# harrywaugh/UOB_Raytracer

Measured on AMD Instinct MI355X. Metric: Mrays/sec (nominal = W*H*AA*(1+S)/t), Cornell Box 4096^2, 8xAA, 64 shadow rays, higher is better.
Workload: dtype f32; 1 GPU; headline: Cornell Box 4096x4096, 4x2 AA, 64 shadow rays, 2 spheres, <=10 bounces, 26 triangles; parallelism=1 GPU

## Files before the change

include/uob_rt.h:

```cpp
#ifndef UOB_RT_H
#define UOB_RT_H

#include <stddef.h>
#include <stdint.h>

#ifdef __cplusplus
extern "C" {
#endif

#define RT_ABI_VERSION 2
#define RT_MAX_SPHERES 4
#define RT_MAX_DEVICES 8

enum {
  RT_OK = 0,
  RT_E_INVALID = -1,
  RT_E_DEVICE = -2,
  RT_E_NOMEM = -3,
  RT_E_IO = -4,
  RT_E_UNSUPPORTED = -5
};

typedef struct rt_sphere {
  float center[3];
// ... 197 lines not shown
int rt_debug_block_costs(rt_ctx* ctx, uint32_t* out, int32_t cap);

int rt_debug_world_masks(rt_ctx* ctx, uint64_t* out, int64_t cap, int32_t* grid, int32_t* words);

int rt_debug_tile_data(rt_ctx* ctx, int32_t* orig, float* tiles, int32_t cap_tiles);

int rt_debug_scene_data(rt_ctx* ctx, float* vertices4, float* normals4, float* colors4, float* vertices4_m,
                        float* normals4_m, float* colors4_m, int32_t* n_shadow, float vbox_lo[3], float vbox_hi[3],
                        int32_t cap_triangles);

int rt_register_output(rt_ctx* ctx, void* host, size_t bytes);
int rt_unregister_output(rt_ctx* ctx);

int rt_debug_wave_timeline(rt_ctx* ctx, uint64_t out[8]);

int rt_debug_wave_seeds(rt_ctx* ctx, void* records, int64_t cap, int32_t dims[3], uint64_t counters[4]);

int rt_debug_wave_seeds_wide(rt_ctx* ctx, void* records, int64_t cap, int32_t dims[3], uint64_t counters[10]);

enum { RT_COPY_2D = 0,
       RT_COPY_PEER = 1,
       RT_COPY_LINEAR = 2    };
typedef struct rt_band_copy {
  int32_t op, reserved;
  uint64_t dst_offset, dst_pitch, src_offset, src_pitch, width_bytes, rows;
} rt_band_copy;
int rt_debug_band_copy_plan(int32_t num_devices, int32_t k, int32_t device_band_rows, int32_t width, int32_t height,
                            int32_t elem_bytes, int32_t dev_to_dev, int32_t peer_ok, int32_t same_device,
                            rt_band_copy* out, int32_t cap);

// ... 35 lines not shown
```

uob_raytracer_amd/csrc/rt_api.hip:

```cpp
#include <cmath>
#include <cstdarg>
#include <cstdio>
#include <cstdlib>
#include <cstring>
#include <memory>
#include <new>
#include <string>
#include <vector>

#include "rt_host.h"

namespace uobrt {

static thread_local std::string g_last_error;

void set_error(const char* fmt, ...) {
  char buf[1024];
  va_list ap;
  va_start(ap, fmt);
  vsnprintf(buf, sizeof buf, fmt, ap);
  va_end(ap);
  g_last_error = buf;
}

// ... 306 lines not shown
  const float zero3[3] = {0.f, 0.f, 0.f}, ident[12] = {1, 0, 0, 0, 0, 1, 0, 0, 0, 0, 1, 0};
  fill_params(c, ident, zero3, light, 1.0f, P);
  if (tiled) use_tiled_scene(c, P);
}

enum class Family { wave, mesh, generic };

static bool frame_cull(const rt_ctx* c) { return !(c->cfg.flags & RT_FLAG_NO_CULL); }

static Family frame_family(const rt_ctx* c, const FrameParams& P) {
  if (c->cfg.flags & RT_FLAG_GENERIC_KERNEL) return Family::generic;
  if (wave_kernel_supports(P) && (frame_cull(c) || P.aa_x * P.aa_y <= 64)) return Family::wave;
  return frame_cull(c) && mesh_kernel_supports(P) ? Family::mesh : Family::generic;
}

static void attach_heavy_lists(rt_ctx* c, FrameParams* P) {
  if (!c->d_heavy_flags || P->job_tasks < 4) return;
  const int prev = c->heavy_phase, cur = prev ^ 1;
  unsigned int* const st[2] = {c->d_jobctr, c->d_jobctr + (2 * kJobHeads + 1) * kJobHeadStride};
  P->heavy_prev = c->d_heavy[prev]; P->heavy_prev_state = st[prev];
  P->heavy_new = c->d_heavy[cur]; P->heavy_new_state = st[cur];
  P->heavy_flags = c->d_heavy_flags + (size_t)prev * c->heavy_jobs_max; P->heavy_flags_new = c->d_heavy_flags + (size_t)cur * c->heavy_jobs_max;
  P->heavy_gen = ++c->heavy_gen;
  P->heavy_factor4 = c->tune.heavy_factor4;
  P->heavy_cap = P->njobs / 3 < c->heavy_cap ? P->njobs / 3 : c->heavy_cap;
  P->heavy_dilate = c->tune.heavy_dilate ? 1 : 0;
  c->heavy_phase = cur;
}

static int attach_timeline(rt_ctx* c, hipStream_t stream, FrameParams* P) {
  c->timeline_valid = false;
  if (!c->tune.timeline) return RT_OK;
  const size_t waves = (size_t)P->wave_blocks * 4;
  if (!c->d_timeline) {
    if (c->d_timeline.alloc(waves * 3) != hipSuccess) { set_error("hipMalloc failed (timeline)"); return RT_E_NOMEM; }
    c->timeline_waves = waves;
  }
  if (c->timeline_waves >= waves) {
    HIP_TRY(hipMemsetAsync(c->d_timeline, 0, c->timeline_waves * 3 * sizeof(uint64_t), stream));
    P->counters = reinterpret_cast<unsigned long long*>(c->d_timeline.p);
    c->timeline_valid = true;
  }
// ... 26 lines not shown
    }
  if (!(fabsf(focal) <= 1.0e9f)) { set_error("focal length must be finite and <= 1e9"); return RT_E_INVALID; }
  for (int k = 0; k < 12; ++k)
    if (!(fabsf(rot[k]) <= 4.0f)) { set_error("rotation matrix entries must be finite and <= 4"); return RT_E_INVALID; }
  if (c->owned_rows == 0) return RT_OK;
  FrameParams P;
  fill_params(c, rot, cam, light, focal, &P);
  P.out_argb = d_argb; P.out_rgb = d_rgb; P.counters = nullptr;
  P.out_global = out_global ? 1 : 0;
  HIP_TRY(hipSetDevice(c->device));
  if (c->timed && stream != c->last_stream) HIP_TRY(hipStreamWaitEvent(stream, c->ev1, 0));
  HIP_TRY(wait_aov(c, stream));
  HIP_TRY(wait_scene(c, stream));
  HIP_TRY(hipEventRecord(c->ev0, stream));
  c->seed_tile_rows = 0;
  const Family family = frame_family(c, P);
  if (family == Family::wave) {
    attach_heavy_lists(c, &P);
    int rc = attach_timeline(c, stream, &P);
    if (rc == RT_OK) rc = attach_seeds(c, rot, &P);
    if (rc != RT_OK) return rc;
    launch_wave(P, frame_cull(c), false, false, stream);
  } else if (family == Family::mesh) {
    use_tiled_scene(c, &P);
    if (c->d_mesh_cost) {
      P.mesh_order = c->mesh_order_valid ? c->d_mesh_order : nullptr;
      P.mesh_cost = c->d_mesh_cost; P.mesh_order_out = c->d_mesh_order;
      P.mesh_queue_len = c->d_mesh_order + 4 * (size_t)((c->cfg.width + 15) / 16) * (size_t)((c->owned_rows + 15) / 16);
      c->mesh_order_valid = true;
    }
    launch_stage_records(P, stream);
    launch_mesh(P, false, false, stream, c->aux_stream, c->ev_fork, c->ev_join);
  } else {
    launch_generic(P, false, stream);
// ... 273 lines not shown
  HIP_TRY(hipMemcpy(rec.data(), c->d_timeline, rec.size() * sizeof(uint64_t), hipMemcpyDeviceToHost));
  for (int q = 0; q < 8; ++q) out[q] = 0;
  out[1] = ~0ull;
  for (size_t w = 0; w < c->timeline_waves; ++w) {
    const uint64_t t0 = rec[3 * w], t1 = rec[3 * w + 1], jobs = rec[3 * w + 2] & 0xffffffffull;
    if (t1 == 0) continue;
    out[7] = rec[3 * w + 2] >> 32;
    out[0] += 1; out[3] += t0; out[4] += t1; out[5] += jobs;
    if (t0 < out[1]) out[1] = t0;
    if (t1 > out[2]) out[2] = t1;
    if (jobs > out[6]) out[6] = jobs;
  }
  return RT_OK;
}

static int seed_table_view(rt_ctx* c, void* records, int64_t cap, int32_t dims[3], uint64_t* counters, int ncounters,
                           void (*view)(SeedRec& r, uint64_t rows, uint64_t* counters)) {
  if (!c || !dims || !counters || cap < 0 || (cap > 0 && !records)) { set_error("NULL argument"); return RT_E_INVALID; }
  c = lead_ctx(c);
  dims[0] = c->seed_tile_rows; dims[1] = c->seed_nseg; dims[2] = c->seed_rows;
  for (int q = 0; q < ncounters; ++q) counters[q] = 0;
  if (c->seed_tile_rows == 0) { dims[1] = 0; return RT_OK; }
  DeviceGuard guard;
  HIP_TRY(hipSetDevice(c->device));
  if (c->timed) HIP_TRY(hipEventSynchronize(c->ev1));
  std::vector<SeedRec> rec((size_t)c->seed_tile_rows * (size_t)c->seed_nseg);
  HIP_TRY(hipMemcpy(rec.data(), c->d_seed, rec.size() * sizeof(SeedRec), hipMemcpyDeviceToHost));
  const rt_config& g = c->cfg;
  for (int tr = 0; tr < c->seed_tile_rows; ++tr) {
    uint64_t rows = 0;
// ... 155 lines not shown
```

uob_raytracer_amd/csrc/rt_device.h:

```cpp
#pragma once
#include <hip/hip_runtime.h>
#include <stdint.h>

#include "../../include/uob_rt.h"

namespace uobrt {

constexpr int kJobHeads = 31;
constexpr int kJobHeadStride = 32;
constexpr int kHeavyStateWords = 8;
constexpr float kMaxCoordinate = 65536.0f;
constexpr int kRecordsPerTriangle = 8;

struct DevSphere {
  float cx, cy, cz, r2;
  float col[4];
};

struct alignas(16) SeedRec {
  float D0[3], ed;
  unsigned long long K, Kh, Kp;
  int32_t h;
  uint32_t flags;
  uint32_t pad[4];
};
// ... 101 lines not shown
```

uob_raytracer_amd/csrc/rt_host.h:

```cpp
#pragma once
#include <hip/hip_runtime.h>

#include <atomic>
#include <string>
#include <utility>
#include <vector>

#include "rt_device.h"

#define HIP_TRY(expr)                                                                   \
  do {                                                                                  \
    hipError_t e_ = (expr);                                                             \
    if (e_ != hipSuccess) {                                                             \
      uobrt::set_error("%s failed: %s (%s:%d)", #expr, hipGetErrorString(e_), __FILE__, __LINE__); \
      return RT_E_DEVICE;                                                               \
    }                                                                                   \
  } while (0)

namespace uobrt {

void set_error(const char* fmt, ...);

struct KeepError {
  std::string text;
// ... 1 lines not shown
  ~KeepError();
};

constexpr int kMaxTriangles = 4000000;
constexpr int kWorldGrid = 32;

void launch_generic(const FrameParams& P, bool count, hipStream_t stream);
bool generic_needs_records(int n);
void launch_stage_records(const FrameParams& P, hipStream_t stream);
void launch_trace_rays(const FrameParams& P, int what, const float* d_rays, const float* d_r2, long nray, int* d_tri,
                       float* d_out10, hipStream_t stream);
void launch_wave(const FrameParams& P, bool cull, bool count, bool prof, hipStream_t stream);
bool wave_kernel_supports(const FrameParams& P);
bool wave_takes_seed(const FrameParams& P, bool cull);
bool wave_can_count(const FrameParams& P, bool cull);
int wave_blocks_per_cu(bool leave_room);
void launch_mesh(const FrameParams& P, bool count, bool prof, hipStream_t stream, hipStream_t aux, hipEvent_t ev_fork, hipEvent_t ev_join);
void launch_bin_primary(const FrameParams& P, hipStream_t stream);
bool mesh_kernel_supports(const FrameParams& P);
int mesh_tiles(int n);
int mesh_occ_words(int grid);
int mesh_screen_cells(int pixels);
int mesh_blocks_per_cu();
int launch_scene_check(const float4* v, const float4* col, int n, unsigned int* out, hipStream_t stream);
void launch_scene_refit(const float4* v, const float4* nrm, const float4* col, const int* orig, int n, float4* vm, float4* nm,
                        float4* cm, float4* tile_box, hipStream_t stream);
constexpr unsigned int kPoseStatic = 0xffffu;
void launch_pose(const float4* rest_v, const float4* rest_n, const unsigned short* object_of, const float* d_xforms12, int n,
                 float4* out_v, float4* out_n, hipStream_t stream);
void launch_skin(const float4* rest_v, const float4* rest_n, const ushort4* index, const float4* weights, const float* d_bones12,
// ... 149 lines not shown
  int cap = 0;
  uobrt::SceneStore own;
  uobrt::DevBuffer tile_scratch;
  int owned_rows = 0;
  uobrt::DevMem<float4> d_verts, d_normals, d_colors;
  uobrt::DevMem<uint32_t> d_argb;
  uobrt::DevMem<float4> d_rgb;
  uobrt::DevMem<unsigned long long> d_counters;
  uobrt::DevMem<unsigned int> d_jobctr;
  uobrt::DevMem<uobrt::SeedRec> d_seed;
  size_t seed_cap = 0;
  int seed_tile_rows = 0, seed_nseg = 0, seed_rows = 0;
  int cus = 256;
  unsigned int *d_heavy[2] = {nullptr, nullptr}, *d_heavy_flags = nullptr;
  int heavy_cap = 0, heavy_phase = 0;
  size_t heavy_jobs_max = 0;
  char* reg_host = nullptr; char* reg_dev = nullptr; size_t reg_bytes = 0;
  bool reg_owner = false;
  bool timeline_valid = false;
  uobrt::DevMem<uint64_t> d_timeline;
  size_t timeline_waves = 0;
  uint32_t heavy_gen = 0;
  float4* d_records = nullptr;
  float4 *d_verts_m = nullptr, *d_normals_m = nullptr, *d_colors_m = nullptr, *d_tile_box = nullptr;
  int* d_orig = nullptr;
  uobrt::DevMem<uobrt::DevSphere> d_spheres;
  unsigned int *d_mesh_cost = nullptr, *d_mesh_order = nullptr;
  bool mesh_order_valid = false;
  unsigned long long *d_screen_masks = nullptr, *d_world_masks = nullptr;
  unsigned int* d_world_occ = nullptr;
// ... 71 lines not shown
```

uob_raytracer_amd/csrc/rt_kernel_wave.hip:

```cpp
#define RT_SPHERES_IN_LDS
#define RT_RNG_JUMP_IN_LDS
#include "rt_host.h"
#include "rt_wave_common.h"

#include <type_traits>
#include <utility>

namespace uobrt {

namespace {

constexpr int kChunk = 4;

struct WaveLds {
  float4* r0;
  float4* r1;
  float2* r2;
  float4* h0;
  float4* h1;
  uint32_t* rng;
};
__host__ __device__ constexpr int wave_lds_bytes(bool cull) {
  return (cull ? 0 : 64 * (16 + 16 + 8)) + 64 * 32 + kRngPixels * kRngStride * 4;
}
// ... 312 lines not shown
  const bool timeline = !COUNT && !PROF && PC(counters) != nullptr;
  unsigned long long* const tls = reinterpret_cast<unsigned long long*>(L.rng + kRngStride + 256);
  if (timeline && lane == 0) { tls[0] = __builtin_amdgcn_s_memrealtime(); tls[1] = 0ull; }
  bool phase_a = n_heavy != 0u;
  const int grid_waves = (int)gridDim.x * kWavesPerBlock;
  const int per_wave = PC(job_tasks) * PT > 32 ? 8 * grid_waves : grid_waves;
  int next_job = -1, chunk_left = 0;
  unsigned int listed = 0u;
  int chunk = PC(njobs) > 2 * per_wave ? kChunk : (PC(njobs) > per_wave ? 2 : 1);
  for (;;) {
  int job = 0;
  const int jt = PC(job_tasks);
  if (phase_a) {
    if (lane == 0) job = (int)atomicAdd(PC(job_counter) + (kJobHeads + head) * kJobHeadStride, 1u);
    const unsigned int unit = (unsigned int)__builtin_amdgcn_readfirstlane(job) * kJobHeads + (unsigned int)head;
    if (unit >= n_heavy) { phase_a = false; continue; }
    job = (int)PC(heavy_prev)[unit];
    if (job < 0 || job >= PC(njobs)) continue;
  } else {
    if (chunk_left > 0) {
      job = next_job; next_job += kJobHeads; --chunk_left; listed >>= 1;
    } else {
      if (lane == 0) job = (int)atomicAdd(PC(job_counter) + head * kJobHeadStride, (unsigned int)chunk);
      job = __builtin_amdgcn_readfirstlane(job) * kJobHeads + head;
      next_job = job + kJobHeads; chunk_left = chunk - 1;
      listed = 0u;
      if (n_heavy != 0u) {
        const int jl = job + lane * kJobHeads;
        listed = (unsigned int)ballot(lane <= chunk_left && jl < PC(njobs) && PC(heavy_flags)[jl] == PC(heavy_gen));
      }
      const int left = PC(njobs) - next_job;
      chunk = left > 2 * per_wave ? kChunk : (left > per_wave ? 2 : 1);
    }
    if (job >= PC(njobs)) {
      chunk_left = 0;
      const unsigned int at = lane < kJobHeads ? __hip_atomic_load(PC(job_counter) + lane * kJobHeadStride, __ATOMIC_RELAXED, __HIP_MEMORY_SCOPE_AGENT) : 0u;
      const unsigned long long avail = ballot(lane < kJobHeads && (long long)at * kJobHeads + lane < (long long)PC(njobs));
      if (avail == 0ull) break;
      const unsigned long long above = avail & ~((2ull << head) - 1ull);
      head = __builtin_ctzll(above != 0ull ? above : avail);
      continue;
    }
    if ((listed & 1u) != 0u) continue;
  }
// ... 311 lines not shown
        if (rel >= 0 && rel < PT) outc = v;
      }
    }
    RT_STAMP(prof, 6)
  }
  const int x = x0 + lane;
  if (!COUNT && !PROF && (BIGAA ? lane < JP : lane < jt * PT) && x < P.W) {
    const f3 c = pixel_colour(outc, aa_full, inv_aa);
    const size_t o = (size_t)(PC(out_global) ? y : lr) * P.W + x;
    PC(out_argb)[o] = pack_argb(c);
    if (PC(out_rgb)) PC(out_rgb)[o] = make_float4(c.x, c.y, c.z, 1.0f);
  }
  if (lpt) {
    const unsigned long long cost = __builtin_amdgcn_s_memtime() - job_t0;
    if (lane == 0) { cost_acc[0] += cost; cost_acc[1] += (unsigned long long)jt; }
    if (cost > heavy_thr * (unsigned long long)jt && lane < (PC(heavy_dilate) ? 3 : 1)) {
      const int jn = job + (lane == 1 ? -1 : (lane == 2 ? 1 : 0));
      const int col = jn - jrow * PC(nseg);
      if (col >= 0 && col < PC(nseg)) {
        const unsigned int was = atomicMax(PC(heavy_flags_new) + jn, PC(heavy_gen) + 1u);
        if (was < PC(heavy_gen) + 1u) {
          const unsigned int at = atomicAdd(PC(heavy_new_state), 1u);
          if (at < (unsigned int)PC(heavy_cap)) PC(heavy_new)[at] = (unsigned int)jn;
          else atomicExch(PC(heavy_flags_new) + jn, was);
        }
      }
    }
  }
  }
  if (lpt && lane == 0) {
    atomicAdd(reinterpret_cast<unsigned long long*>(PC(heavy_new_state) + 2), cost_acc[0]);
    atomicAdd(PC(heavy_new_state) + 4, (unsigned int)cost_acc[1]);
  }
  if (timeline && lane == 0) {
    const unsigned long long t1 = __builtin_amdgcn_s_memrealtime(), t0 = tls[0];
    unsigned long long* const rec = PC(counters) + 3 * (size_t)(blockIdx.x * kWavesPerBlock + wave);
    rec[0] = t0; rec[1] = t1; rec[2] = tls[1] | ((unsigned long long)n_heavy << 32);
  }
  if (PROF) {
// ... 172 lines not shown
static const WaveVariant& wave_frame_variant(const FrameParams& P, bool cull) { return kWaveVariants[wave_choose(P, {cull, false, false})].v; }

template <size_t I>
static void launch_variant(const FrameParams& P, dim3 grid, hipStream_t stream) {
  constexpr WaveVariant v = kWaveVariants[I].v;
  hipLaunchKernelGGL((rt_draw_wave<v.cull, v.count, v.prof, v.stride, v.multi, v.aa_x, v.aa_y, v.ss, v.bigaa>), grid,
                     dim3(64 * kWavesPerBlock), static_lds(v) ? 0 : wave_kernel_lds(P, v.cull), stream, P);
}
template <size_t... I>
static void launch_chosen(size_t i, const FrameParams& P, dim3 grid, hipStream_t stream, std::index_sequence<I...>) {
  ((i == I ? launch_variant<I>(P, grid, stream) : void()), ...);
}

bool wave_takes_seed(const FrameParams& P, bool cull) { return takes_seed(wave_frame_variant(P, cull)) && P.job_tasks == 8; }

bool wave_can_count(const FrameParams& P, bool cull) { return has_counting_build(wave_frame_variant(P, cull)); }

void launch_wave(const FrameParams& P, bool cull, bool count, bool prof, hipStream_t stream) {
  if (P.seed != nullptr && !count)
    hipLaunchKernelGGL(rt_wave_seed, wave_grid(P, P.seed_tile_rows * P.nseg), dim3(64 * kWavesPerBlock), wave_kernel_lds(P, true), stream, P);
  const size_t heads_bytes = 2 * kJobHeads * kJobHeadStride * sizeof(unsigned int), state_bytes = kJobHeadStride * sizeof(unsigned int);
  if (P.heavy_new != nullptr && !count) {
    const bool before = P.heavy_new_state < P.job_counter;
    hipMemsetAsync(before ? (void*)P.heavy_new_state : (void*)P.job_counter, 0, heads_bytes + state_bytes, stream);
  } else {
    hipMemsetAsync(P.job_counter, 0, heads_bytes, stream);
  }
  launch_chosen(wave_choose(P, {cull, count, prof}), P, wave_grid(P, P.njobs), stream, std::make_index_sequence<kNumWaveVariants>{});
}

// ... 2 lines not shown
```

uob_raytracer_amd/csrc/rt_scene.hip:

```cpp
#include <cmath>
#include <cstring>
#include <vector>

#include "rt_host.h"

using namespace uobrt;

int uobrt::validate_spheres(const rt_sphere* sph, int num) {
  for (int i = 0; i < num; ++i) {
    const rt_sphere& s = sph[i];
    for (int k = 0; k < 3; ++k)
      if (!(fabsf(s.center[k]) <= kMaxCoordinate)) { set_error("sphere %d: |centre| must be finite and <= 2^16", i); return RT_E_INVALID; }
    if (!(fabsf(s.radius_sq) <= kMaxCoordinate * kMaxCoordinate)) { set_error("sphere %d: radius_sq must be finite and <= 2^32", i); return RT_E_INVALID; }
  }
  return RT_OK;
}

int uobrt::validate_vertices(const float* vertices4, int n) {
  for (size_t k = 0; k < (size_t)n * 12; ++k) {
    if ((k & 3) != 3 && !(fabsf(vertices4[k]) <= kMaxCoordinate)) {
      set_error("vertex %zu: coordinates must be finite and |x| <= 2^16", k / 4); return RT_E_INVALID;
    }
  }
  return RT_OK;
// ... 119 lines not shown
  const bool grow = n > c->cap || !c->d_verts;
  const size_t cap = grow ? (n > 0 ? n : 1) : c->cap;
  if (grow) {
    fresh.cap = (int)cap;
    get(fresh.verts, 3 * cap); get(fresh.normals, cap); get(fresh.colors, cap);
    if (q.records || o.records) get(fresh.t.records, cap * kRecordsPerTriangle);
    if (q.tiled || o.verts_m) tiled_set(&fresh.t, cap);
    if (q.masks || o.screen_masks) mask_set(&fresh.t, cap);
  } else {
    if (q.records && !o.records) get(o.records, cap * kRecordsPerTriangle);
    if (q.tiled && !o.verts_m) tiled_set(&o, cap);
    if (q.masks && !o.screen_masks) mask_set(&o, cap);
  }
  if (q.masks && !o.world_occ) get(o.world_occ, (size_t)mesh_occ_words(kWorldGrid));
  if (q.heavy && !o.heavy_flags) {
    get(o.heavy[0], (size_t)c->heavy_cap); get(o.heavy[1], (size_t)c->heavy_cap); get(o.heavy_flags, 2 * c->heavy_jobs_max);
  }
  if (q.mesh_sched && !o.mesh_cost) {
    const size_t jobs = (size_t)((cfg.width + 15) / 16) * (size_t)((c->owned_rows + 15) / 16);
    get(o.mesh_cost, jobs ? jobs : 1); get(o.mesh_order, 4 * (jobs ? jobs : 1) + 1);
  }
  if (!ok) return alloc_failed();
  if (device_tiles && q.tiled) {
    const int rc = ensure_bytes(&c->tile_scratch, tile_build_scratch_bytes((int)cap));
    if (rc != RT_OK) return rc;
  }
  if (q.masks && !c->aux_stream &&
      (c->aux_stream.create(hipStreamNonBlocking) != hipSuccess || c->ev_fork.create(hipEventDisableTiming) != hipSuccess ||
       c->ev_join.create(hipEventDisableTiming) != hipSuccess)) {
    set_error("stream/event creation failed"); return RT_E_DEVICE;
  }
// ... 40 lines not shown
  c->d_colors_m = q.tiled ? o.colors_m : nullptr; c->d_orig = q.tiled ? o.orig : nullptr; c->d_tile_box = q.tiled ? o.tile_box : nullptr;
  c->d_screen_masks = q.masks ? o.screen_masks : nullptr; c->d_world_masks = q.masks ? o.world_masks : nullptr;
  c->d_world_occ = q.masks ? o.world_occ : nullptr;
  c->nwords = q.masks ? (mesh_tiles(n) + 63) / 64 : 0;
  c->scx = q.masks ? mesh_screen_cells(c->cfg.width) : 0; c->scy = q.masks ? mesh_screen_cells(c->cfg.height) : 0;
  c->d_heavy[0] = q.heavy ? o.heavy[0] : nullptr; c->d_heavy[1] = q.heavy ? o.heavy[1] : nullptr;
  c->d_heavy_flags = q.heavy ? o.heavy_flags : nullptr;
  c->d_mesh_cost = q.mesh_sched ? o.mesh_cost : nullptr; c->d_mesh_order = q.mesh_sched ? o.mesh_order : nullptr;
}

static int scene_switch(rt_ctx* c, int n, bool first, hipStream_t s) {
  const bool restart = first || (c->n > 64) != (n > 64);
  scene_select(c, n);
  if (!restart) return RT_OK;
  c->mesh_order_valid = false;
  c->heavy_phase = 0; c->heavy_gen = 0;
  HIP_TRY(hipMemsetAsync(c->d_jobctr, 0, (2 * kJobHeads + 2) * kJobHeadStride * sizeof(unsigned int), s));
  if (c->d_heavy_flags) HIP_TRY(hipMemsetAsync(c->d_heavy_flags, 0, 2 * c->heavy_jobs_max * 4, s));
  return RT_OK;
}

struct SceneEdit {
  const void *v, *nr, *col;
  bool on_device;
  int n;
  bool replace, first;
  uint32_t flags;
  hipStream_t s;
  SceneSummary sum;
};

// ... 466 lines not shown
```

uob_raytracer_amd/csrc/rt_wave_common.h:

```cpp
#pragma once
#include "rt_trace.h"

namespace uobrt {
namespace {

constexpr int kRngPixels = 4;
constexpr int kRngStride = 64 * 4 + 4;

__device__ __forceinline__ float rl(float v, int lane) {
  return __int_as_float(__builtin_amdgcn_readlane(__float_as_int(v), lane));
}
__device__ __forceinline__ float shfl(float v, int lane) { return __shfl(v, lane, 64); }
__device__ __forceinline__ int opaque(int v) {
  asm volatile("" : "+v"(v));
  return v;
}
__device__ __forceinline__ unsigned long long ballot(bool p) { return __builtin_amdgcn_ballot_w64(p); }
__device__ __forceinline__ float norm1(f3 a) { return fabsf(a.x) + fabsf(a.y) + fabsf(a.z); }
__device__ __forceinline__ float bsqrt(float x) { return __builtin_amdgcn_sqrtf(x); }
__device__ __forceinline__ float norm_inf(f3 a) { return fmaxf(fmaxf(fabsf(a.x), fabsf(a.y)), fabsf(a.z)); }
__device__ __forceinline__ float max_abs3(float a, float b, float c) { return fmaxf(fmaxf(fabsf(a), fabsf(b)), fabsf(c)); }

typedef const __attribute__((address_space(4))) FrameParams* KernargParams;
__device__ __forceinline__ KernargParams cold(const FrameParams&) {
  unsigned long long a = (unsigned long long)__builtin_amdgcn_kernarg_segment_ptr();
  asm volatile("" : "+s"(a));
  return (KernargParams)a;
}
__device__ __forceinline__ int band_global_row_cold(const FrameParams& P, int lr) {
  KernargParams K = cold(P);
  const int br = K->band_rows;
  const int q = (int)div_magic((uint32_t)lr, K->band_rows_magic);
  return (q * K->band_count + K->band_index) * br + (lr - q * br);
}
#define PC(field) (cold(P)->field)

constexpr int kRngSegs = 5, kRngSegLen = 13;
struct RngJumpTable { uint32_t col[kRngSegs - 1][32]; };
constexpr uint32_t xorshift_c(uint32_t s) { s ^= s << 13; s ^= s >> 17; s ^= s << 5; return s; }
constexpr RngJumpTable make_rng_jump_table() {
  RngJumpTable t{};
  for (int g = 1; g < kRngSegs; ++g)
    for (int b = 0; b < 32; ++b) {
      uint32_t v = 1u << b;
      for (int k = 0; k < kRngSegLen * g; ++k) v = xorshift_c(v);
      t.col[g - 1][b] = v;
    }
  return t;
}
__constant__ const RngJumpTable kRngJump = make_rng_jump_table();
// ... 491 lines not shown
```

uob_raytracer_amd/runtime.py:

```python
import ctypes as C
import os

import numpy as np

try:
    import torch as _torch
except ImportError:
    _torch = None

from . import abi

_HERE = os.path.dirname(os.path.abspath(__file__))
LIB_PATH = os.environ.get("UOB_RT_LIB", os.path.join(_HERE, "libuob_rt.so"))

EXPORTS = (
    "rt_abi_version", "rt_last_error", "rt_config_default", "rt_config_owned_rows", "rt_init", "rt_render",
    "rt_render_device", "rt_count_work", "rt_count_executed", "rt_last_kernel_ms", "rt_destroy", "rt_scene_cornell_box",
    "rt_scene_load_obj", "rt_scene_load_obj_ex", "rt_triangle_compute_normal", "rt_scene_pack", "rt_rotation_matrix",
    "rt_selftest_rcp", "rt_selftest_normalize", "rt_selftest_shade", "rt_selftest_all_within", "rt_debug_trace_rays", "rt_debug_block_costs", "rt_debug_world_masks", "rt_debug_wave_timeline", "rt_debug_wave_seeds", "rt_debug_wave_seeds_wide", "rt_register_output", "rt_unregister_output",
    "rt_debug_band_copy_plan", "rt_update_scene", "rt_update_scene_device", "rt_debug_tile_data",
    "rt_trace_rays", "rt_trace_rays_device", "rt_debug_trace_stats",
    "rt_render_aov", "rt_render_aov_device", "rt_debug_aov_stats",
    "rt_shade_points", "rt_shade_points_device", "rt_debug_shade_stats",
    "rt_radiance_rays", "rt_radiance_rays_device", "rt_debug_radiance_stats",
    "rt_replace_scene", "rt_replace_scene_device", "rt_update_spheres", "rt_debug_scene_capacity",
    "rt_scene_transform", "rt_set_objects", "rt_pose_objects", "rt_pose_objects_device", "rt_debug_object_count",
    "rt_debug_scene_data",
    "rt_scene_skin", "rt_set_skin", "rt_pose_skin", "rt_pose_skin_device", "rt_debug_skin_info",
    "rt_debug_live_device_objects",
    "rt_filter_params_default", "rt_filter_plane", "rt_filter_plane_device", "rt_debug_filter_stats", "rt_filter_plane_host",
    "rt_accumulate_params_default", "rt_accumulate_plane", "rt_accumulate_plane_device", "rt_debug_accumulate_stats",
    "rt_accumulate_plane_host",
    "rt_motion_snapshot", "rt_motion_release", "rt_debug_motion_info", "rt_motion_planes", "rt_motion_planes_device",
    "rt_motion_planes_host", "rt_debug_motion_stats",
# ... 105 lines not shown
        L.rt_debug_accumulate_stats.argtypes = [vp, C.POINTER(C.c_uint64)]
        L.rt_accumulate_plane_host.argtypes = [ap, fp, fp, fp, ip, fp, fp, fp, fp]
        L.rt_motion_snapshot.argtypes = [vp, vp]
        L.rt_motion_release.argtypes = [vp]
        L.rt_debug_motion_info.argtypes = [vp, ip]
        L.rt_motion_planes.argtypes = [vp, ip, fp, fp, C.c_int64, fp, fp]
        L.rt_motion_planes_device.argtypes = [vp, vp, vp, vp, C.c_int64, vp, vp, vp]
        L.rt_motion_planes_host.argtypes = [fp, fp, fp, C.c_int32, ip, fp, fp, C.c_int64, fp, fp]
        L.rt_debug_motion_stats.argtypes = [vp, C.POINTER(C.c_uint64)]
        L.rt_accumulate_plane_moving.argtypes = [vp, ap, fp, fp, fp, ip, fp, fp, fp, fp, fp, fp]
        L.rt_accumulate_plane_moving_device.argtypes = [vp, ap] + [vp] * 11
        L.rt_accumulate_plane_moving_host.argtypes = [ap, fp, fp, fp, ip, fp, fp, fp, fp, fp, fp]
        L.rt_debug_block_costs.argtypes = [vp, C.POINTER(C.c_uint32), C.c_int32]
        L.rt_debug_world_masks.argtypes = [vp, C.POINTER(C.c_uint64), C.c_int64, C.POINTER(C.c_int32), C.POINTER(C.c_int32)]
        L.rt_debug_wave_timeline.argtypes = [vp, C.POINTER(C.c_uint64)]
        L.rt_debug_band_copy_plan.argtypes = [C.c_int32] * 9 + [C.POINTER(abi.RtBandCopy), C.c_int32]
        L.rt_register_output.argtypes = [vp, vp, C.c_size_t]
        L.rt_unregister_output.argtypes = [vp]
        L.rt_triangle_compute_normal.argtypes = [C.POINTER(abi.RtTriangle)]
        L.rt_triangle_compute_normal.restype = None
        L.rt_scene_pack.argtypes = [C.POINTER(abi.RtTriangle), C.c_int32, fp, fp, fp]
        L.rt_scene_pack.restype = None
        L.rt_rotation_matrix.argtypes = [C.c_float, C.c_float, fp]
        L.rt_rotation_matrix.restype = None
        if L.rt_abi_version() != abi.RT_ABI_VERSION:
            raise ImportError("libuob_rt.so ABI %d != binding %d" % (L.rt_abi_version(), abi.RT_ABI_VERSION))
        _lib = L
    return _lib


# ... 46 lines not shown
        raise ValueError("value must be a torch tensor of shape [height, width]")
    h, w = value.shape
    _need("value", value, _torch.float32, (h, w), dev)
    _need("position4", position4, _torch.float32, (h, w, 4), dev)
    _need("normal4", normal4, _torch.float32, (h, w, 4), dev)
    return h, w


def _seeds_ptr(seeds, k, what):
    if seeds is None:
        return None
    seeds = np.ascontiguousarray(seeds, np.int32).reshape(-1)
    if seeds.shape[0] != k:
        raise ValueError("seeds must have one entry per %s" % what)
    return seeds.ctypes.data_as(C.POINTER(C.c_int32))


def band_copy_plan(num_devices, k, device_band_rows, width, height, elem_bytes, dev_to_dev, peer_ok, same_device):
    n = _check(lib().rt_debug_band_copy_plan(num_devices, k, device_band_rows, width, height, elem_bytes, int(dev_to_dev),
                                             int(peer_ok), int(same_device), None, 0))
    buf = (abi.RtBandCopy * max(n, 1))()
    _check(lib().rt_debug_band_copy_plan(num_devices, k, device_band_rows, width, height, elem_bytes, int(dev_to_dev),
                                         int(peer_ok), int(same_device), buf, n))
    return [{f: int(getattr(buf[i], f)) for f, _ in abi.RtBandCopy._fields_ if f != "reserved"} for i in range(n)]


def live_device_objects():
    out = (C.c_int64 * 4)()
    _check(lib().rt_debug_live_device_objects(out))
    return {key: int(out[i]) for i, key in enumerate(LIVE_OBJECT_KEYS)}
# ... 877 lines not shown
        rays = torch.cat([start, d], -1).reshape(-1, 6).contiguous()
        seeds = (torch.arange(width * height, dtype=torch.int64, device=dev) & abi.RT_SHADE_SEED_MASK).to(torch.int32)
        return self.radiance_rays_device(rays, light, seeds=seeds).reshape(height, width, 4)

    def trace_stats(self):
        return self._stats("rt_debug_trace_stats", TRACE_STATS_KEYS)

    def wave_timeline(self):
        out = (C.c_uint64 * 8)()
        _check(lib().rt_debug_wave_timeline(self._h, out))
        n = max(int(out[0]), 1)
        first, last = int(out[1]), int(out[2])
        return {"waves": int(out[0]), "span_us": (last - first) / 100.0, "mean_start_us": (int(out[3]) / n - first) / 100.0,
                "mean_idle_tail_us": (last - int(out[4]) / n) / 100.0, "jobs": int(out[5]), "max_jobs_per_wave": int(out[6]), "listed_jobs": int(out[7])}

    def _wave_seed_records(self, export, ncounters):
        fn = getattr(lib(), export)
        fn.argtypes = [C.c_void_p, C.c_void_p, C.c_int64, C.POINTER(C.c_int32), C.POINTER(C.c_uint64)]
        dims, cnt = (C.c_int32 * 3)(), (C.c_uint64 * ncounters)()
        _check(fn(self._h, None, 0, dims, cnt))
        rec = np.zeros((int(dims[0]), int(dims[1])), SEED_DTYPE)
        if rec.size:
            _check(fn(self._h, rec.ctypes.data_as(C.c_void_p), rec.size, dims, cnt))
        return {"tile_rows": int(dims[0]), "tiles_per_row": int(dims[1]), "rows_per_tile": int(dims[2]), "records": rec}, cnt

    def wave_seeds(self):
        d, cnt = self._wave_seed_records("rt_debug_wave_seeds", 4)
        d.update(tiles_primary=int(cnt[0]), tiles_shadow=int(cnt[1]), jobs_primary=int(cnt[2]), jobs_shadow=int(cnt[3]))
        return d

# ... 24 lines not shown
```

Baseline: 4.413 million Mrays/s.

## Bucket expensive wave jobs into cost classes and dispatch costliest first

Measured per-job cost is now sorted into three geometric cost classes, not a single heavy flag. The heavy-job list is split per class so the next frame's phase A hands out the most expensive class first, a longest-processing-time style ordering meant to shrink the idle tail at the end of the persistent wave kernel. Flag words now pack generation and class, with a periodic flag reset when the generation counter would overflow. Debug exports are added for inspecting the lists. In exchange there are extra atomics per heavy job and a larger heavy-list allocation.

```diff
diff --git a/include/uob_rt.h b/include/uob_rt.h
--- a/include/uob_rt.h
+++ b/include/uob_rt.h
@@ -235,6 +235,12 @@
 
 int rt_debug_wave_timeline(rt_ctx* ctx, uint64_t out[8]);
 
+int rt_debug_wave_heavy(rt_ctx* ctx, int32_t* entry_jobs, int32_t* entry_classes, int64_t entries_cap, int32_t* job_flag_classes,
+                        int64_t jobs_cap, int64_t info[16]);
+
+int rt_debug_heavy_order(const uint64_t* costs, int64_t ncosts, uint64_t thr, uint32_t job_tasks, int32_t* cost_class,
+                         const uint32_t* counts, uint32_t cap, int64_t nunits, int32_t* unit_class, uint32_t* unit_index);
+
 int rt_debug_wave_seeds(rt_ctx* ctx, void* records, int64_t cap, int32_t dims[3], uint64_t counters[4]);
 
 int rt_debug_wave_seeds_wide(rt_ctx* ctx, void* records, int64_t cap, int32_t dims[3], uint64_t counters[10]);
diff --git a/uob_raytracer_amd/csrc/rt_api.hip b/uob_raytracer_amd/csrc/rt_api.hip
--- a/uob_raytracer_amd/csrc/rt_api.hip
+++ b/uob_raytracer_amd/csrc/rt_api.hip
@@ -344,8 +344,13 @@
   return frame_cull(c) && mesh_kernel_supports(P) ? Family::mesh : Family::generic;
 }
 
-static void attach_heavy_lists(rt_ctx* c, FrameParams* P) {
-  if (!c->d_heavy_flags || P->job_tasks < 4) return;
+static int attach_heavy_lists(rt_ctx* c, hipStream_t stream, FrameParams* P) {
+  c->heavy_last_jobs = 0;
+  if (!c->d_heavy_flags || P->job_tasks < 4) return RT_OK;
+  if (c->heavy_gen >= kHeavyGenMax) {
+    HIP_TRY(hipMemsetAsync(c->d_heavy_flags, 0, 2 * c->heavy_jobs_max * sizeof(unsigned int), stream));
+    c->heavy_gen = 0;
+  }
   const int prev = c->heavy_phase, cur = prev ^ 1;
   unsigned int* const st[2] = {c->d_jobctr, c->d_jobctr + (2 * kJobHeads + 1) * kJobHeadStride};
   P->heavy_prev = c->d_heavy[prev]; P->heavy_prev_state = st[prev];
@@ -356,6 +361,8 @@
   P->heavy_cap = P->njobs / 3 < c->heavy_cap ? P->njobs / 3 : c->heavy_cap;
   P->heavy_dilate = c->tune.heavy_dilate ? 1 : 0;
   c->heavy_phase = cur;
+  c->heavy_last_jobs = P->njobs; c->heavy_last_cap = P->heavy_cap;
+  return RT_OK;
 }
 
 static int attach_timeline(rt_ctx* c, hipStream_t stream, FrameParams* P) {
@@ -412,10 +419,11 @@
   HIP_TRY(wait_scene(c, stream));
   HIP_TRY(hipEventRecord(c->ev0, stream));
   c->seed_tile_rows = 0;
+  c->heavy_last_jobs = 0;
   const Family family = frame_family(c, P);
   if (family == Family::wave) {
-    attach_heavy_lists(c, &P);
-    int rc = attach_timeline(c, stream, &P);
+    int rc = attach_heavy_lists(c, stream, &P);
+    if (rc == RT_OK) rc = attach_timeline(c, stream, &P);
     if (rc == RT_OK) rc = attach_seeds(c, rot, &P);
     if (rc != RT_OK) return rc;
     launch_wave(P, frame_cull(c), false, false, stream);
@@ -719,6 +727,55 @@
   return RT_OK;
 }
 
+int rt_debug_heavy_order(const uint64_t* costs, int64_t ncosts, uint64_t thr, uint32_t job_tasks, int32_t* cost_class,
+                         const uint32_t* counts, uint32_t cap, int64_t nunits, int32_t* unit_class, uint32_t* unit_index) {
+  if (ncosts < 0 || nunits < 0 || nunits > 0xffffffffll || (ncosts > 0 && (!costs || !cost_class)) ||
+      (nunits > 0 && (!counts || !unit_class || !unit_index))) {
+    set_error("rt_debug_heavy_order: NULL argument or a count out of range"); return RT_E_INVALID;
+  }
+  for (int64_t i = 0; i < ncosts; ++i) cost_class[i] = wave_heavy_class(costs[i], thr, job_tasks);
+  for (int64_t u = 0; u < nunits; ++u) unit_class[u] = wave_heavy_slot(counts, cap, (unsigned int)u, &unit_index[u]);
+  return kHeavyClasses;
+}
+
+int rt_debug_wave_heavy(rt_ctx* c, int32_t* entry_jobs, int32_t* entry_classes, int64_t entries_cap, int32_t* job_flag_classes,
+                        int64_t jobs_cap, int64_t info[16]) {
+  if (!c || !info || entries_cap < 0 || jobs_cap < 0 || (entries_cap > 0 && (!entry_jobs || !entry_classes)) ||
+      (jobs_cap > 0 && !job_flag_classes)) {
+    set_error("rt_debug_wave_heavy: NULL argument"); return RT_E_INVALID;
+  }
+  c = lead_ctx(c);
+  if (!c->d_heavy_flags || c->heavy_last_jobs == 0) {
+    set_error("rt_debug_wave_heavy: the context's last frame built no expensive-job list"); return RT_E_UNSUPPORTED;
+  }
+  DeviceGuard guard;
+  HIP_TRY(hipSetDevice(c->device));
+  if (c->timed) HIP_TRY(hipEventSynchronize(c->ev1));
+  const int cur = c->heavy_phase;
+  const size_t cap = (size_t)c->heavy_last_cap, njobs = (size_t)c->heavy_last_jobs;
+  unsigned int state[kJobHeadStride];
+  HIP_TRY(hipMemcpy(state, cur == 0 ? c->d_jobctr : c->d_jobctr + (2 * kJobHeads + 1) * kJobHeadStride, sizeof state, hipMemcpyDeviceToHost));
+  std::vector<unsigned int> list((size_t)kHeavyClasses * cap), flags(njobs);
+  if (!list.empty()) HIP_TRY(hipMemcpy(list.data(), c->d_heavy[cur], list.size() * sizeof(unsigned int), hipMemcpyDeviceToHost));
+  HIP_TRY(hipMemcpy(flags.data(), c->d_heavy_flags + (size_t)cur * c->heavy_jobs_max, njobs * sizeof(unsigned int), hipMemcpyDeviceToHost));
+  for (int q = 0; q < 16; ++q) info[q] = 0;
+  info[0] = kHeavyClasses; info[1] = (int64_t)cap; info[3] = (int64_t)njobs; info[4] = state[0];
+  const unsigned int gen = c->heavy_gen + 1u;
+  int64_t n = 0;
+  for (unsigned int u = 0;; ++u) {
+    unsigned int index;
+    const int cls = wave_heavy_slot(state + kHeavyClassWord, (unsigned int)cap, u, &index);
+    if (cls < 0) break;
+    if (n < entries_cap) { entry_jobs[n] = (int32_t)list[(size_t)cls * cap + index]; entry_classes[n] = cls; }
+    ++n;
+    info[8 + cls] += 1;
+  }
+  info[2] = n;
+  for (size_t j = 0; j < njobs && (int64_t)j < jobs_cap; ++j)
+    job_flag_classes[j] = (flags[j] >> kHeavyClassBits) == gen ? (int32_t)(flags[j] & ((1u << kHeavyClassBits) - 1u)) : -1;
+  return RT_OK;
+}
+
 static int seed_table_view(rt_ctx* c, void* records, int64_t cap, int32_t dims[3], uint64_t* counters, int ncounters,
                            void (*view)(SeedRec& r, uint64_t rows, uint64_t* counters)) {
   if (!c || !dims || !counters || cap < 0 || (cap > 0 && !records)) { set_error("NULL argument"); return RT_E_INVALID; }
diff --git a/uob_raytracer_amd/csrc/rt_device.h b/uob_raytracer_amd/csrc/rt_device.h
--- a/uob_raytracer_amd/csrc/rt_device.h
+++ b/uob_raytracer_amd/csrc/rt_device.h
@@ -9,6 +9,13 @@
 constexpr int kJobHeads = 31;
 constexpr int kJobHeadStride = 32;
 constexpr int kHeavyStateWords = 8;
+constexpr int kHeavyClasses = 3;
+constexpr int kHeavyClassShift = 1;
+constexpr int kHeavyClassWord = 8;
+constexpr int kHeavyClassBits = 3;
+constexpr unsigned int kHeavyGenMax = (1u << (32 - kHeavyClassBits)) - 2u;
+static_assert(kHeavyClasses >= 1 && kHeavyClasses <= (1 << kHeavyClassBits), "a class must fit in its bits of the flag word");
+static_assert(kHeavyClassWord >= kHeavyStateWords && kHeavyClassWord + kHeavyClasses <= kJobHeadStride, "the class counts lie in the state's line");
 constexpr float kMaxCoordinate = 65536.0f;
 constexpr int kRecordsPerTriangle = 8;
 
diff --git a/uob_raytracer_amd/csrc/rt_host.h b/uob_raytracer_amd/csrc/rt_host.h
--- a/uob_raytracer_amd/csrc/rt_host.h
+++ b/uob_raytracer_amd/csrc/rt_host.h
@@ -39,6 +39,8 @@
 bool wave_kernel_supports(const FrameParams& P);
 bool wave_takes_seed(const FrameParams& P, bool cull);
 bool wave_can_count(const FrameParams& P, bool cull);
+int wave_heavy_class(unsigned long long cost, unsigned long long thr, unsigned int job_tasks);
+int wave_heavy_slot(const unsigned int* counts, unsigned int cap, unsigned int unit, unsigned int* index);
 int wave_blocks_per_cu(bool leave_room);
 void launch_mesh(const FrameParams& P, bool count, bool prof, hipStream_t stream, hipStream_t aux, hipEvent_t ev_fork, hipEvent_t ev_join);
 void launch_bin_primary(const FrameParams& P, hipStream_t stream);
@@ -218,6 +220,7 @@
   int cus = 256;
   unsigned int *d_heavy[2] = {nullptr, nullptr}, *d_heavy_flags = nullptr;
   int heavy_cap = 0, heavy_phase = 0;
+  int heavy_last_jobs = 0, heavy_last_cap = 0;
   size_t heavy_jobs_max = 0;
   char* reg_host = nullptr; char* reg_dev = nullptr; size_t reg_bytes = 0;
   bool reg_owner = false;
diff --git a/uob_raytracer_amd/csrc/rt_kernel_wave.hip b/uob_raytracer_amd/csrc/rt_kernel_wave.hip
--- a/uob_raytracer_amd/csrc/rt_kernel_wave.hip
+++ b/uob_raytracer_amd/csrc/rt_kernel_wave.hip
@@ -350,9 +350,11 @@
   if (phase_a) {
     if (lane == 0) job = (int)atomicAdd(PC(job_counter) + (kJobHeads + head) * kJobHeadStride, 1u);
     const unsigned int unit = (unsigned int)__builtin_amdgcn_readfirstlane(job) * kJobHeads + (unsigned int)head;
-    if (unit >= n_heavy) { phase_a = false; continue; }
-    job = (int)PC(heavy_prev)[unit];
+    const HeavySlot at = heavy_slot(PC(heavy_prev_state) + kHeavyClassWord, (unsigned int)PC(heavy_cap), unit);
+    if (at.cls < 0) { phase_a = false; continue; }
+    job = (int)PC(heavy_prev)[(size_t)at.cls * (size_t)PC(heavy_cap) + at.index];
     if (job < 0 || job >= PC(njobs)) continue;
+    if (PC(heavy_flags)[job] != ((PC(heavy_gen) << kHeavyClassBits) | (unsigned int)at.cls)) continue;
   } else {
     if (chunk_left > 0) {
       job = next_job; next_job += kJobHeads; --chunk_left; listed >>= 1;
@@ -363,7 +365,8 @@
       listed = 0u;
       if (n_heavy != 0u) {
         const int jl = job + lane * kJobHeads;
-        listed = (unsigned int)ballot(lane <= chunk_left && jl < PC(njobs) && PC(heavy_flags)[jl] == PC(heavy_gen));
+        listed = (unsigned int)ballot(lane <= chunk_left && jl < PC(njobs) &&
+                                      PC(heavy_flags)[jl] - (PC(heavy_gen) << kHeavyClassBits) < (unsigned int)kHeavyClasses);
       }
       const int left = PC(njobs) - next_job;
       chunk = left > 2 * per_wave ? kChunk : (left > per_wave ? 2 : 1);
@@ -705,15 +708,17 @@
   if (lpt) {
     const unsigned long long cost = __builtin_amdgcn_s_memtime() - job_t0;
     if (lane == 0) { cost_acc[0] += cost; cost_acc[1] += (unsigned long long)jt; }
-    if (cost > heavy_thr * (unsigned long long)jt && lane < (PC(heavy_dilate) ? 3 : 1)) {
+    const int cls = heavy_class(cost, heavy_thr, (unsigned int)jt);
+    if (cls >= 0 && lane < (PC(heavy_dilate) ? 3 : 1)) {
       const int jn = job + (lane == 1 ? -1 : (lane == 2 ? 1 : 0));
       const int col = jn - jrow * PC(nseg);
       if (col >= 0 && col < PC(nseg)) {
-        const unsigned int was = atomicMax(PC(heavy_flags_new) + jn, PC(heavy_gen) + 1u);
-        if (was < PC(heavy_gen) + 1u) {
+        const unsigned int mine = ((PC(heavy_gen) + 1u) << kHeavyClassBits) | (unsigned int)cls;
+        unsigned int* const flag = PC(heavy_flags_new) + jn;
+        if (__hip_atomic_load(flag, __ATOMIC_RELAXED, __HIP_MEMORY_SCOPE_AGENT) < mine) {
           const unsigned int at = atomicAdd(PC(heavy_new_state), 1u);
-          if (at < (unsigned int)PC(heavy_cap)) PC(heavy_new)[at] = (unsigned int)jn;
-          else atomicExch(PC(heavy_flags_new) + jn, was);
+          if (at < (unsigned int)PC(heavy_cap) && atomicMax(flag, mine) < mine)
+            PC(heavy_new)[(size_t)cls * (size_t)PC(heavy_cap) + atomicAdd(PC(heavy_new_state) + kHeavyClassWord + cls, 1u)] = (unsigned int)jn;
         }
       }
     }
@@ -916,6 +921,13 @@
 
 bool wave_takes_seed(const FrameParams& P, bool cull) { return takes_seed(wave_frame_variant(P, cull)) && P.job_tasks == 8; }
 
+int wave_heavy_class(unsigned long long cost, unsigned long long thr, unsigned int job_tasks) { return heavy_class(cost, thr, job_tasks); }
+int wave_heavy_slot(const unsigned int* counts, unsigned int cap, unsigned int unit, unsigned int* index) {
+  const HeavySlot s = heavy_slot(counts, cap, unit);
+  *index = s.index;
+  return s.cls;
+}
+
 bool wave_can_count(const FrameParams& P, bool cull) { return has_counting_build(wave_frame_variant(P, cull)); }
 
 void launch_wave(const FrameParams& P, bool cull, bool count, bool prof, hipStream_t stream) {
diff --git a/uob_raytracer_amd/csrc/rt_scene.hip b/uob_raytracer_amd/csrc/rt_scene.hip
--- a/uob_raytracer_amd/csrc/rt_scene.hip
+++ b/uob_raytracer_amd/csrc/rt_scene.hip
@@ -157,7 +157,8 @@
   }
   if (q.masks && !o.world_occ) get(o.world_occ, (size_t)mesh_occ_words(kWorldGrid));
   if (q.heavy && !o.heavy_flags) {
-    get(o.heavy[0], (size_t)c->heavy_cap); get(o.heavy[1], (size_t)c->heavy_cap); get(o.heavy_flags, 2 * c->heavy_jobs_max);
+    get(o.heavy[0], (size_t)kHeavyClasses * c->heavy_cap); get(o.heavy[1], (size_t)kHeavyClasses * c->heavy_cap);
+    get(o.heavy_flags, 2 * c->heavy_jobs_max);
   }
   if (q.mesh_sched && !o.mesh_cost) {
     const size_t jobs = (size_t)((cfg.width + 15) / 16) * (size_t)((c->owned_rows + 15) / 16);
@@ -228,7 +229,7 @@
   scene_select(c, n);
   if (!restart) return RT_OK;
   c->mesh_order_valid = false;
-  c->heavy_phase = 0; c->heavy_gen = 0;
+  c->heavy_phase = 0; c->heavy_gen = 0; c->heavy_last_jobs = 0;
   HIP_TRY(hipMemsetAsync(c->d_jobctr, 0, (2 * kJobHeads + 2) * kJobHeadStride * sizeof(unsigned int), s));
   if (c->d_heavy_flags) HIP_TRY(hipMemsetAsync(c->d_heavy_flags, 0, 2 * c->heavy_jobs_max * 4, s));
   return RT_OK;
diff --git a/uob_raytracer_amd/csrc/rt_wave_common.h b/uob_raytracer_amd/csrc/rt_wave_common.h
--- a/uob_raytracer_amd/csrc/rt_wave_common.h
+++ b/uob_raytracer_amd/csrc/rt_wave_common.h
@@ -34,6 +34,26 @@
   return (q * K->band_count + K->band_index) * br + (lr - q * br);
 }
 #define PC(field) (cold(P)->field)
+
+__host__ __device__ __forceinline__ int heavy_class(unsigned long long cost, unsigned long long thr, unsigned int jt) {
+  if (cost == 0ull || jt == 0u || thr > ~0ull / jt) return -1;
+  const unsigned long long T = thr * jt, c1 = cost - 1ull;
+  int q = -1;
+#pragma unroll
+  for (int k = 0; k < kHeavyClasses; ++k)
+    if ((c1 >> (k * kHeavyClassShift)) >= T) q = k;
+  return q;
+}
+struct HeavySlot { int cls; unsigned int index; };
+__host__ __device__ __forceinline__ HeavySlot heavy_slot(const unsigned int* counts, unsigned int cap, unsigned int unit) {
+#pragma unroll
+  for (int q = kHeavyClasses - 1; q >= 0; --q) {
+    const unsigned int c = counts[q] < cap ? counts[q] : cap;
+    if (unit < c) return HeavySlot{q, unit};
+    unit -= c;
+  }
+  return HeavySlot{-1, 0u};
+}
 
 constexpr int kRngSegs = 5, kRngSegLen = 13;
 struct RngJumpTable { uint32_t col[kRngSegs - 1][32]; };
diff --git a/uob_raytracer_amd/runtime.py b/uob_raytracer_amd/runtime.py
--- a/uob_raytracer_amd/runtime.py
+++ b/uob_raytracer_amd/runtime.py
@@ -17,7 +17,7 @@
     "rt_abi_version", "rt_last_error", "rt_config_default", "rt_config_owned_rows", "rt_init", "rt_render",
     "rt_render_device", "rt_count_work", "rt_count_executed", "rt_last_kernel_ms", "rt_destroy", "rt_scene_cornell_box",
     "rt_scene_load_obj", "rt_scene_load_obj_ex", "rt_triangle_compute_normal", "rt_scene_pack", "rt_rotation_matrix",
-    "rt_selftest_rcp", "rt_selftest_normalize", "rt_selftest_shade", "rt_selftest_all_within", "rt_debug_trace_rays", "rt_debug_block_costs", "rt_debug_world_masks", "rt_debug_wave_timeline", "rt_debug_wave_seeds", "rt_debug_wave_seeds_wide", "rt_register_output", "rt_unregister_output",
+    "rt_selftest_rcp", "rt_selftest_normalize", "rt_selftest_shade", "rt_selftest_all_within", "rt_debug_trace_rays", "rt_debug_block_costs", "rt_debug_world_masks", "rt_debug_wave_timeline", "rt_debug_wave_heavy", "rt_debug_heavy_order", "rt_debug_wave_seeds", "rt_debug_wave_seeds_wide", "rt_register_output", "rt_unregister_output",
     "rt_debug_band_copy_plan", "rt_update_scene", "rt_update_scene_device", "rt_debug_tile_data",
     "rt_trace_rays", "rt_trace_rays_device", "rt_debug_trace_stats",
     "rt_render_aov", "rt_render_aov_device", "rt_debug_aov_stats",
@@ -153,6 +153,9 @@
         L.rt_debug_block_costs.argtypes = [vp, C.POINTER(C.c_uint32), C.c_int32]
         L.rt_debug_world_masks.argtypes = [vp, C.POINTER(C.c_uint64), C.c_int64, C.POINTER(C.c_int32), C.POINTER(C.c_int32)]
         L.rt_debug_wave_timeline.argtypes = [vp, C.POINTER(C.c_uint64)]
+        L.rt_debug_wave_heavy.argtypes = [vp, ip, ip, C.c_int64, ip, C.c_int64, C.POINTER(C.c_int64)]
+        L.rt_debug_heavy_order.argtypes = [C.POINTER(C.c_uint64), C.c_int64, C.c_uint64, C.c_uint32, ip, C.POINTER(C.c_uint32),
+                                           C.c_uint32, C.c_int64, ip, C.POINTER(C.c_uint32)]
         L.rt_debug_band_copy_plan.argtypes = [C.c_int32] * 9 + [C.POINTER(abi.RtBandCopy), C.c_int32]
         L.rt_register_output.argtypes = [vp, vp, C.c_size_t]
         L.rt_unregister_output.argtypes = [vp]
@@ -229,6 +232,20 @@
     if seeds.shape[0] != k:
         raise ValueError("seeds must have one entry per %s" % what)
     return seeds.ctypes.data_as(C.POINTER(C.c_int32))
+
+
+def heavy_order(costs=(), thr=0, job_tasks=1, counts=None, cap=0, nunits=0):
+    costs = np.ascontiguousarray(costs, np.uint64).reshape(-1)
+    cc = np.zeros(max(len(costs), 1), np.int32)
+    uc, ui = np.zeros(max(nunits, 1), np.int32), np.zeros(max(nunits, 1), np.uint32)
+    cnt = np.ascontiguousarray(counts if counts is not None else [0], np.uint32).reshape(-1)
+    if len(cnt) < _check(lib().rt_debug_heavy_order(None, 0, 0, 1, None, None, 0, 0, None, None)):
+        if counts is not None or nunits:
+            raise ValueError("counts must hold one entry per class")
+    q = _check(lib().rt_debug_heavy_order(costs.ctypes.data_as(C.POINTER(C.c_uint64)), len(costs), int(thr), int(job_tasks), _ip(cc),
+                                          cnt.ctypes.data_as(C.POINTER(C.c_uint32)), int(cap), int(nunits), _ip(uc),
+                                          ui.ctypes.data_as(C.POINTER(C.c_uint32))))
+    return q, cc[:len(costs)], uc[:nunits], ui[:nunits]
 
 
 def band_copy_plan(num_devices, k, device_band_rows, width, height, elem_bytes, dev_to_dev, peer_ok, same_device):
@@ -1136,6 +1153,17 @@
         return {"waves": int(out[0]), "span_us": (last - first) / 100.0, "mean_start_us": (int(out[3]) / n - first) / 100.0,
                 "mean_idle_tail_us": (last - int(out[4]) / n) / 100.0, "jobs": int(out[5]), "max_jobs_per_wave": int(out[6]), "listed_jobs": int(out[7])}
 
+    def wave_heavy(self):
+        info = (C.c_int64 * 16)()
+        _check(lib().rt_debug_wave_heavy(self._h, None, None, 0, None, 0, info))
+        n, jobs = int(info[2]), int(info[3])
+        ej, ec, fl = np.zeros(max(n, 1), np.int32), np.zeros(max(n, 1), np.int32), np.zeros(max(jobs, 1), np.int32)
+        _check(lib().rt_debug_wave_heavy(self._h, _ip(ej), _ip(ec), n, _ip(fl), jobs, info))
+        q = int(info[0])
+        return {"classes": q, "cap": int(info[1]), "jobs": jobs, "asked": int(info[4]),
+                "counts": [int(info[8 + k]) for k in range(q)], "entry_jobs": ej[:n], "entry_classes": ec[:n],
+                "job_flag_classes": fl[:jobs]}
+
     def _wave_seed_records(self, export, ncounters):
         fn = getattr(lib(), export)
         fn.argtypes = [C.c_void_p, C.c_void_p, C.c_int64, C.POINTER(C.c_int32), C.POINTER(C.c_uint64)]
```

Result: no change. 4.427 million Mrays/s, median of 6 (+0.3%).
